# bgconley/cadence-rag

Hardware: AMD Instinct MI355X
Metric: queries/sec @ recall@10=1.0 (exact cosine top-10, 1024-d fp32 corpus) (higher is better)
Workload: dtype f32; 1 GPU; BASELINE configs[1]: brute-force cosine top-10, 100000x1024 fp32 corpus on one GPU, 64 queries/step resident in HBM; rows_per_gpu=100000, rows_total=100000, dim=1024, k=10, parallelism=1 GPU, rounds=1, arithmetic=fp16-MFMA prefilter (proven bound) + exact fp32 rescoring, api=crag_index_search_async (in stream order), hbm_bytes_per_corpus_row=6156

## Files before the change

### cadence_rag_amd/csrc/crag_api.hip

```cpp

#include <hip/hip_runtime.h>
#include <stdarg.h>
#include <stdint.h>
#include <stdio.h>
#include <stdlib.h>
#include <string.h>

#include <mutex>
#include <new>
#include <vector>

#include "../../include/crag_dense.h"
#include "crag_kernels.h"

namespace {

thread_local char g_err[512] = "";

int fail(int code, const char *fmt, ...) {
    va_list ap;
    va_start(ap, fmt);
    vsnprintf(g_err, sizeof(g_err), fmt, ap);
    va_end(ap);
    return code;
}

#define HIP_TRY(expr)                                                                          \
    do {                                                                                       \
        hipError_t e_ = (expr);                                                                \
        if (e_ != hipSuccess)                                                                  \
            return fail(CRAG_EHIP, "%s failed: %s (%s:%d)", #expr, hipGetErrorString(e_),      \
                        __FILE__, __LINE__);                                                   \
    } while (0)

bool is_device_ptr(const void *p) {
    if (!p) return false;
    hipPointerAttribute_t attr;
    memset(&attr, 0, sizeof(attr));
    hipError_t e = hipPointerGetAttributes(&attr, p);
    if (e != hipSuccess) {
        (void)hipGetLastError();
        return false;
    }
    return attr.type == hipMemoryTypeDevice || attr.type == hipMemoryTypeManaged;
}

struct DevBuf {
    void *p = nullptr;
    size_t bytes = 0;
    int ensure(size_t need) {
        if (need <= bytes) return CRAG_OK;
        if (p) (void)hipFree(p);
        p = nullptr;
        bytes = 0;
        size_t want = need + need / 4;
        hipError_t e = hipMalloc(&p, want);
        if (e != hipSuccess) {
            p = nullptr;
            return fail(CRAG_ENOMEM, "hipMalloc(%zu) failed: %s", want, hipGetErrorString(e));
        }
        bytes = want;
        return CRAG_OK;
    }
    void release() {
        if (p) (void)hipFree(p);
        p = nullptr;
        bytes = 0;
    }
};

struct EvSet {
    hipEvent_t e0, e1a, e1, e2, e3;
};

}

struct crag_index {
    int device = 0;
    int dim = 0;
    int64_t capacity = 0;
    int64_t cap_rows = 0;
    int64_t size = 0;
    int n_cu = 0;
    float *corpus = nullptr;
    _Float16 *corpus16 = nullptr;
    float *inv_norm = nullptr;
    int64_t *ids = nullptr;
    static constexpr int MAX_WS = 8;
    struct Workspace {
        hipStream_t stream = nullptr;
        bool in_use = false;
        DevBuf partial, gbound;
        DevBuf a32, a16, qinv, pf_gbound, pf_cand, pf_count, pf_flags, pf_xkeys, pf_xids, pf_xcount, pf_xticket;
        hipEvent_t done = nullptr;
        uint32_t seq = 0;
        bool done_recorded = false;
        bool dirty = false;
        uint64_t last_use = 0;
    } ws[MAX_WS];
    static constexpr int MAX_PIPE = 4;
    int n_pipe = 3;
    hipStream_t pipe[MAX_PIPE] = {nullptr, nullptr, nullptr, nullptr};
    hipEvent_t pipe_fork[MAX_PIPE] = {nullptr, nullptr, nullptr, nullptr}, pipe_done[MAX_PIPE] = {nullptr, nullptr, nullptr, nullptr};
    bool pipe_pending[MAX_PIPE] = {false, false, false, false};
    unsigned pipe_next = 0;
    uint64_t use_clock = 0;
    bool record_done = false;
    int64_t last_id = INT64_MIN;
    bool env_no_wide = false, env_no_reverse = false, env_unpipelined = false, env_no_prefilter = false, env_no_rsplit = false;
    int env_pf_derive_lag = 2, env_pf_read_lag = 4;
    int env_pf_nt = -1;
    int64_t nt_above_bytes = 1536ll << 20;
    bool irregular = false;
    uint32_t *irregular_dev = nullptr;
    unsigned long long *pf_stats = nullptr;
    unsigned long long *phase_trace = nullptr;
    const char *last_scan_kernel = "";
    DevBuf stage_q, stage_rows, stage_ids, stage_mask, stage_out, scratch;
    int64_t edit_chunk_rows = 16384;
    DevBuf edit_bounce, edit_srcpos, edit_mask, edit_prefix, edit_newpos;
    std::mutex mu;
    int pass_parity = 0;
    int64_t env_fail_after_scan = 0;
    int64_t pf_searches = 0;
    int profiling = 0;
    int64_t prof_calls = 0;
    std::vector<EvSet> ev_pool;
    size_t ev_used = 0;
};

static_assert(crag_index::MAX_WS == crag::PF_STAT_WS, "one block of statistics records per workspace");

namespace {

struct DeviceGuard {
    int prev = -1;
    bool ok = false;
    explicit DeviceGuard(int dev) {
        if (hipGetDevice(&prev) != hipSuccess) prev = -1;
        ok = (hipSetDevice(dev) == hipSuccess);
    }
    ~DeviceGuard() {
        if (prev >= 0) (void)hipSetDevice(prev);
    }
};

int scan_groups(const crag_index *ix) {
    int64_t n8 = (ix->size + 7) / 8;
    int64_t g = ix->n_cu;
    if (g > n8) g = n8;
    if (g < 1) g = 1;
    return (int)g;
}

int search_device(crag_index *ix, const float *d_queries, int nq, int k, const uint8_t *d_mask,
                  int64_t mask_stride, int64_t *d_out_ids, float *d_out_scores, int32_t *d_out_counts,
                  hipStream_t st) {
    if (nq <= 0) return CRAG_OK;
    int q_blocks = (nq + 31) / 32;
    const bool wide = (nq > 32) && !ix->env_no_wide;
    if (wide) q_blocks = ((nq + 63) / 64) * 2;
    const int nq_pad = q_blocks * 32;
    const int G = scan_groups(ix);
    const bool prefilter = !ix->env_no_prefilter && !ix->irregular &&
                           ix->size >= (int64_t)G * crag::PF_MIN_ROWS_PER_GROUP && (wide || nq <= 32);
    int rc;
    crag_index::Workspace *ws = nullptr;
    for (auto &w : ix->ws)
        if (w.in_use && w.stream == st) ws = &w;
    if (!ws)
        for (auto &w : ix->ws)
            if (!w.in_use) {
                w.in_use = true;
                w.stream = st;
                ws = &w;
                if (&w == &ix->ws[crag_index::MAX_WS - 1]) ix->record_done = true;
                break;
            }
    if (!ws) {
        for (auto &w : ix->ws)
            if (!ws || w.last_use < ws->last_use) ws = &w;
        if (ws->done_recorded && !ws->dirty) {
            HIP_TRY(hipStreamWaitEvent(st, ws->done, 0));
        } else {
            HIP_TRY(hipDeviceSynchronize());
        }
        ix->record_done = true;
        ws->stream = st;
    }
    ws->last_use = ++ix->use_clock;
    if ((rc = ws->partial.ensure((size_t)q_blocks * G * 32 * (size_t)k * sizeof(uint2)))) return rc;
    {
        const size_t gb_bytes = (size_t)q_blocks * 32 * crag::GB_CELLS * sizeof(uint32_t);
        if (gb_bytes > ws->gbound.bytes) {
            if ((rc = ws->gbound.ensure(gb_bytes))) return rc;
            HIP_TRY(hipMemsetAsync(ws->gbound.p, 0, ws->gbound.bytes, st));
        }
    }
    if ((rc = ws->a32.ensure((size_t)nq_pad * crag::DIM * sizeof(float)))) return rc;
    if ((rc = ws->qinv.ensure((size_t)nq_pad * sizeof(float)))) return rc;
    const int cap = (k > 104 && nq_pad <= 128) ? 32768 : 8192;
    const int rsplit = (k <= 32 || ix->env_no_rsplit) ? 1 : (nq <= 16 ? 8 : (nq <= 128 ? 4 : 1));
    if (prefilter) {
        if ((rc = ws->a16.ensure((size_t)nq_pad * crag::DIM * 2))) return rc;
        {
            const size_t need = (size_t)(ix->n_cu + nq_pad) * crag::PF_BOUND_CELLS * sizeof(uint32_t);
            if (need > ws->pf_gbound.bytes) {
                if ((rc = ws->pf_gbound.ensure(need))) return rc;
                HIP_TRY(hipMemsetAsync(ws->pf_gbound.p, 0, ws->pf_gbound.bytes, st));
            }
        }
        if ((rc = ws->pf_cand.ensure((size_t)nq_pad * cap * sizeof(uint2)))) return rc;
        if (rsplit > 1) {
            const size_t slots = (size_t)nq_pad * 8;
            if ((rc = ws->pf_xkeys.ensure(slots * CRAG_MAX_K * sizeof(uint64_t)))) return rc;
            if ((rc = ws->pf_xids.ensure(slots * CRAG_MAX_K * sizeof(int64_t)))) return rc;
            if ((rc = ws->pf_xcount.ensure(slots * sizeof(uint2)))) return rc;
            const size_t tneed = (size_t)nq_pad * sizeof(uint32_t);
            if (tneed > ws->pf_xticket.bytes) {
                if ((rc = ws->pf_xticket.ensure(tneed))) return rc;
                HIP_TRY(hipMemsetAsync(ws->pf_xticket.p, 0, ws->pf_xticket.bytes, st));
            }
        }
        {
            const size_t need = (size_t)nq_pad * sizeof(uint32_t);
            if (need > ws->pf_count.bytes) {
                if ((rc = ws->pf_count.ensure(need))) return rc;
                HIP_TRY(hipMemsetAsync(ws->pf_count.p, 0, ws->pf_count.bytes, st));
            }
            if (ws->pf_flags.bytes == 0) {
                if ((rc = ws->pf_flags.ensure(4 * sizeof(uint32_t)))) return rc;
                HIP_TRY(hipMemsetAsync(ws->pf_flags.p, 0, ws->pf_flags.bytes, st));
            }
        }
        if (ws->dirty) {
            HIP_TRY(hipMemsetAsync(ws->pf_gbound.p, 0, ws->pf_gbound.bytes, st));
            HIP_TRY(hipMemsetAsync(ws->pf_count.p, 0, ws->pf_count.bytes, st));
            HIP_TRY(hipMemsetAsync(ws->pf_flags.p, 0, ws->pf_flags.bytes, st));
            if (ws->pf_xticket.p) HIP_TRY(hipMemsetAsync(ws->pf_xticket.p, 0, ws->pf_xticket.bytes, st));
            ws->dirty = false;
        }
    }

    const int64_t rows_per_g = (ix->size + G - 1) / G + 64;
    if (rows_per_g * (int64_t)(crag::DIM * 4) >= (int64_t)0x7ff00000)
        return fail(CRAG_EINVAL, "index too large for one device scan window (%lld rows)",
                    (long long)ix->size);

    EvSet *ev = nullptr;
    if (ix->profiling > 0 && (ix->prof_calls++ % ix->profiling) == ix->profiling / 2) {
        if (ix->ev_used == ix->ev_pool.size()) {
            EvSet t;
            HIP_TRY(hipEventCreate(&t.e0));
            HIP_TRY(hipEventCreate(&t.e1a));
            HIP_TRY(hipEventCreate(&t.e1));
            HIP_TRY(hipEventCreate(&t.e2));
            HIP_TRY(hipEventCreate(&t.e3));
            ix->ev_pool.push_back(t);
        }
        ev = &ix->ev_pool[ix->ev_used++];
        HIP_TRY(hipEventRecord(ev->e0, st));
    }

    crag::PrepParams pp;
    pp.queries = d_queries;
    pp.nq = nq;
    pp.dim = ix->dim;
    pp.qinv = (float *)ws->qinv.p;
    pp.a32 = (float *)ws->a32.p;
    pp.a16 = prefilter ? (_Float16 *)ws->a16.p : nullptr;
    HIP_TRY(crag::launch_prep_queries(pp, nq_pad, st));

    crag::ScanParams sp;
    sp.wide = wide ? 1 : 0;
    sp.corpus = ix->corpus;
    sp.inv_norm = ix->inv_norm;
    sp.queries = d_queries;
    sp.a32 = (const float *)ws->a32.p;
    sp.qinv = (const float *)ws->qinv.p;
    sp.gate = nullptr;
    sp.dim = ix->dim;
    sp.mask = (const uint32_t *)d_mask;
    sp.mask_stride_w = mask_stride / 4;
    sp.partial = (uint2 *)ws->partial.p;
    sp.gbound = (uint32_t *)ws->gbound.p;
    sp.n_rows = ix->size;
    sp.cap_rows = ix->cap_rows;
    sp.nq = nq;
    sp.k = k;
    sp.G = G;
    sp.nb = k < crag::GB_CELLS ? k : crag::GB_CELLS;
    sp.pub_rank = (k + sp.nb - 1) / sp.nb - 1;
    sp.reverse = ix->pass_parity;
    ix->pass_parity ^= 1;
    if (ix->env_no_reverse) sp.reverse = 0;
    sp.unpipelined = (ix->env_unpipelined && !prefilter) ? 1 : 0;
    sp.piece_shift = crag::crag_piece_shift(ix->corpus16 != nullptr);

    crag::MergeParams mp;
    mp.partial = (const uint2 *)ws->partial.p;
    mp.ids = ix->ids;
    mp.gbound = (uint32_t *)ws->gbound.p;
    mp.id_base = 0;
    mp.out_ids = d_out_ids;
    mp.out_scores = d_out_scores;
    mp.out_counts = d_out_counts;
    mp.k = k;
    mp.G = G;

    if (ev) {
        HIP_TRY(hipEventRecord(ev->e1a, st));
        HIP_TRY(hipEventRecord(ev->e1, st));
    }
    if (prefilter) {
        crag::PfParams fp;
        fp.corpus = ix->corpus;
        fp.corpus16 = ix->corpus16;
        fp.inv_norm = ix->inv_norm;
        fp.a16 = (const _Float16 *)ws->a16.p;
        fp.qinv = (const float *)ws->qinv.p;
        fp.mask = (const uint32_t *)d_mask;
        fp.mask_stride_w = mask_stride / 4;
        fp.gbound_idle = (const uint32_t *)ws->pf_gbound.p;
        fp.gbound = (uint32_t *)ws->pf_gbound.p + (size_t)ix->n_cu * crag::PF_BOUND_CELLS;
        fp.cand = (uint2 *)ws->pf_cand.p;
        fp.count = (uint32_t *)ws->pf_count.p;
        fp.flags = (uint32_t *)ws->pf_flags.p;
        if (++ws->seq == 0u) ws->seq = 1u;
        fp.seq = ws->seq;
        fp.n_rows = ix->size;
        fp.nq = nq;
        fp.k = k;
        fp.G = G;
        fp.reverse = sp.reverse;
        fp.sets = k <= 24 ? 1 : (k <= 56 ? 2 : 4);
        fp.pub0 = (k + fp.sets - 1) / fp.sets >= 27 ? 8 : fp.sets;
        fp.cap = cap;
        fp.derive_lag = ix->corpus16 ? ix->env_pf_derive_lag : 1;
        fp.read_lag = ix->corpus16 ? ix->env_pf_read_lag : 2;
        {
            const int64_t streamed = ix->size * (int64_t)crag::DIM * 2;
            fp.nt = !ix->corpus16 ? 0 : (ix->env_pf_nt >= 0 ? ix->env_pf_nt : (streamed > ix->nt_above_bytes ? 1 : 0));
        }
        const int nqb = wide ? 2 : 1;
        ws->dirty = true;
        HIP_TRY(crag::launch_prefilter(fp, nqb, nq_pad / (32 * nqb), st, &ix->last_scan_kernel));
        if (ix->env_fail_after_scan > 0 && ++ix->pf_searches == ix->env_fail_after_scan)
            return fail(CRAG_EHIP, "injected failure behind the scan launch (CRAG_TEST_FAIL_AFTER_SCAN)");
        if (ev) HIP_TRY(hipEventRecord(ev->e2, st));
        crag::FinParams fin;
        fin.corpus = ix->corpus;
        fin.inv_norm = ix->inv_norm;
        fin.a32 = (const float *)ws->a32.p;
        fin.qinv = (const float *)ws->qinv.p;
        fin.cand = (const uint2 *)ws->pf_cand.p;
        fin.count = (uint32_t *)ws->pf_count.p;
        fin.gbound = fp.gbound;
        fin.flags = (const uint32_t *)ws->pf_flags.p;
        fin.seq = fp.seq;
        fin.ids = ix->ids;
        fin.out_ids = d_out_ids;
        fin.out_scores = d_out_scores;
        fin.out_counts = d_out_counts;
        fin.stats = ix->pf_stats + (size_t)(ws - ix->ws) * (crag::PF_STAT_SLOTS / crag_index::MAX_WS) * 3;
        fin.k = k;
        fin.cap = cap;
        fin.merge = mp;
        fin.nq = nq;
        fin.rsplit = rsplit;
        fin.xkeys = nullptr;
        fin.xids = nullptr;
        fin.xcount = nullptr;
        fin.xticket = nullptr;
        if (fin.rsplit > 1) {
            fin.xkeys = (uint64_t *)ws->pf_xkeys.p;
            fin.xids = (int64_t *)ws->pf_xids.p;
            fin.xcount = (uint2 *)ws->pf_xcount.p;
            fin.xticket = (uint32_t *)ws->pf_xticket.p;
        }
        sp.wide = 0;
        sp.gate = nullptr;
        sp.unpipelined = 1;
        fin.scan = sp;
        fin.fb_blocks = G * ((nq + 31) / 32);
        fin.fb_done = (uint32_t *)ws->pf_flags.p + 1;
        fin.trace = ix->phase_trace;
        HIP_TRY(crag::launch_finalize(fin, st));
        ws->dirty = false;
    } else {
        HIP_TRY(crag::launch_scan(sp, q_blocks, st, &ix->last_scan_kernel));
        if (ev) HIP_TRY(hipEventRecord(ev->e2, st));
        HIP_TRY(crag::launch_merge_partials(mp, nq, st));
    }
    if (ev) HIP_TRY(hipEventRecord(ev->e3, st));
    ws->done_recorded = ix->record_done;
    if (ix->record_done) HIP_TRY(hipEventRecord(ws->done, st));
    return CRAG_OK;
}

int check_search_args(const crag_index *ix, const void *queries, int nq, int k, const void *mask,
                      int64_t mask_stride, const void *out_ids, const void *out_scores,
// ... 9 lines not shown
            return fail(CRAG_EINVAL, "mask_stride must be 0 or a multiple of 4 >= %lld (got %lld)",
                        (long long)need, (long long)mask_stride);
        if (((uintptr_t)mask) & 3) return fail(CRAG_EINVAL, "row_mask must be 4-byte aligned");
    }
    return CRAG_OK;
}

}

extern "C" {

const char *crag_last_error(void) { return g_err; }

void crag_set_error_(const char *msg) { snprintf(g_err, sizeof(g_err), "%s", msg ? msg : ""); }

const char *crag_version(void) { return "cadence-rag_amd dense lane 0.1 (gfx950)"; }

int crag_device_count(void) {
    int n = 0;
    if (hipGetDeviceCount(&n) != hipSuccess) {
        (void)hipGetLastError();
        return 0;
    }
    return n;
}

int crag_index_create(int device, int dim, int64_t capacity, crag_index **out) {
    if (!out) return fail(CRAG_EINVAL, "out is NULL");
    *out = nullptr;
    if (dim <= 0 || dim > CRAG_DIM) return fail(CRAG_EINVAL, "dim must be in [1, %d] (got %d)", CRAG_DIM, dim);
    if (capacity <= 0) return fail(CRAG_EINVAL, "capacity must be > 0 (got %lld)", (long long)capacity);
    int ndev = crag_device_count();
    if (ndev <= 0) return fail(CRAG_ENODEV, "no HIP device visible");
    if (device < 0 || device >= ndev) return fail(CRAG_EINVAL, "device %d out of range [0, %d)", device, ndev);
    DeviceGuard guard(device);
    if (!guard.ok) return fail(CRAG_EHIP, "hipSetDevice(%d) failed", device);
    hipDeviceProp_t prop;
    HIP_TRY(hipGetDeviceProperties(&prop, device));
    if (strncmp(prop.gcnArchName, "gfx950", 6) != 0)
        return fail(CRAG_ENODEV, "device %d is %s; this library is built for gfx950 only", device,
                    prop.gcnArchName);
    crag_index *ix = new (std::nothrow) crag_index();
    if (!ix) return fail(CRAG_ENOMEM, "out of host memory");
    ix->device = device;
    ix->dim = dim;
    ix->capacity = capacity;
    ix->cap_rows = ((capacity + 31) / 32) * 32;
    ix->n_cu = prop.multiProcessorCount;
    const size_t cbytes = (size_t)ix->cap_rows * crag::DIM * sizeof(float);
    hipError_t e;
    if ((e = hipMalloc((void **)&ix->corpus, cbytes)) != hipSuccess ||
        (e = hipMalloc((void **)&ix->inv_norm, (size_t)ix->cap_rows * sizeof(float))) != hipSuccess ||
        (e = hipMalloc((void **)&ix->ids, (size_t)ix->cap_rows * sizeof(int64_t))) != hipSuccess) {
        int rc = fail(CRAG_ENOMEM, "hipMalloc for %lld rows failed: %s", (long long)ix->cap_rows,
                      hipGetErrorString(e));
        crag_index_destroy(ix);
        return rc;
    }
    if ((e = hipMemset(ix->inv_norm, 0, (size_t)ix->cap_rows * sizeof(float))) != hipSuccess ||
        (e = hipMemset(ix->corpus, 0, cbytes)) != hipSuccess) {
        int rc = fail(CRAG_EHIP, "hipMemset failed: %s", hipGetErrorString(e));
        crag_index_destroy(ix);
        return rc;
    }
    for (auto &w : ix->ws)
        if ((e = hipEventCreateWithFlags(&w.done, hipEventDisableTiming)) != hipSuccess) {
            int rc = fail(CRAG_EHIP, "hipEventCreate failed: %s", hipGetErrorString(e));
            crag_index_destroy(ix);
            return rc;
        }
    ix->env_no_wide = getenv("CRAG_NO_WIDE") != nullptr;
    ix->env_no_reverse = getenv("CRAG_NO_REVERSE") != nullptr;
    ix->env_unpipelined = getenv("CRAG_UNPIPELINED") != nullptr;
    ix->env_no_prefilter = getenv("CRAG_NO_PREFILTER") != nullptr;
    ix->env_no_rsplit = getenv("CRAG_NO_RSPLIT") != nullptr;
    if (const char *v = getenv("CRAG_PF_NT")) ix->env_pf_nt = atoi(v) ? 1 : 0;
    if (const char *v = getenv("CRAG_PF_LAGS")) {
        int d = 0, r = 0;
        if (sscanf(v, "%d,%d", &d, &r) == 2 && d >= 1 && r > d && r <= 4) {
            ix->env_pf_derive_lag = d;
            ix->env_pf_read_lag = r;
        }
    }
    if (const char *v = getenv("CRAG_TEST_FAIL_AFTER_SCAN")) ix->env_fail_after_scan = atoll(v);
    if (const char *v = getenv("CRAG_PIPE_STREAMS")) {
        const int n = atoi(v);
        if (n >= 1 && n <= crag_index::MAX_PIPE) ix->n_pipe = n;
    }
    if (const char *v = getenv("CRAG_EDIT_CHUNK_ROWS")) {
        const long long c = atoll(v);
        if (c >= 32 && c % 32 == 0 && c <= ((long long)1 << 24)) ix->edit_chunk_rows = c;
    }
    if (const char *v = getenv("CRAG_PF_NT_ABOVE_MB")) ix->nt_above_bytes = (int64_t)atoll(v) << 20;
    if (!ix->env_no_prefilter && getenv("CRAG_NO_FP16_MIRROR") == nullptr) {
        const size_t mbytes = (size_t)ix->cap_rows * crag::DIM * sizeof(_Float16);
        if ((e = hipMalloc((void **)&ix->corpus16, mbytes)) != hipSuccess ||
            (e = hipMemset(ix->corpus16, 0, mbytes)) != hipSuccess) {
            int rc = fail(CRAG_ENOMEM, "hipMalloc for the fp16 mirror of %lld rows failed: %s", (long long)ix->cap_rows,
                          hipGetErrorString(e));
            crag_index_destroy(ix);
            return rc;
        }
    }
    if ((e = hipMalloc((void **)&ix->irregular_dev, sizeof(uint32_t))) != hipSuccess ||
        (e = hipMalloc((void **)&ix->pf_stats, crag::PF_STAT_SLOTS * 3 * sizeof(unsigned long long))) != hipSuccess ||
        (e = hipMemset(ix->irregular_dev, 0, sizeof(uint32_t))) != hipSuccess ||
        (e = hipMemset(ix->pf_stats, 0, crag::PF_STAT_SLOTS * 3 * sizeof(unsigned long long))) != hipSuccess) {
        int rc = fail(CRAG_ENOMEM, "hipMalloc for the index state failed: %s", hipGetErrorString(e));
        crag_index_destroy(ix);
        return rc;
    }
    if (getenv("CRAG_PHASE_TRACE") != nullptr) {
        if ((e = hipMalloc((void **)&ix->phase_trace, 128 * sizeof(unsigned long long))) != hipSuccess ||
            (e = hipMemset(ix->phase_trace, 0, 128 * sizeof(unsigned long long))) != hipSuccess) {
            int rc = fail(CRAG_ENOMEM, "hipMalloc for the phase trace failed: %s", hipGetErrorString(e));
            crag_index_destroy(ix);
            return rc;
        }
    }
    *out = ix;
    return CRAG_OK;
}

int crag_index_destroy(crag_index *ix) {
    if (!ix) return CRAG_OK;
    DeviceGuard guard(ix->device);
    (void)hipDeviceSynchronize();
    for (auto &t : ix->ev_pool) {
        (void)hipEventDestroy(t.e0);
        (void)hipEventDestroy(t.e1a);
        (void)hipEventDestroy(t.e1);
        (void)hipEventDestroy(t.e2);
        (void)hipEventDestroy(t.e3);
    }
    if (ix->irregular_dev) (void)hipFree(ix->irregular_dev);
    if (ix->phase_trace) (void)hipFree(ix->phase_trace);
    for (int i = 0; i < crag_index::MAX_PIPE; ++i) {
        if (ix->pipe_fork[i]) (void)hipEventDestroy(ix->pipe_fork[i]);
        if (ix->pipe_done[i]) (void)hipEventDestroy(ix->pipe_done[i]);
        if (ix->pipe[i]) (void)hipStreamDestroy(ix->pipe[i]);
    }
    if (ix->pf_stats) (void)hipFree(ix->pf_stats);
    if (ix->corpus) (void)hipFree(ix->corpus);
    if (ix->corpus16) (void)hipFree(ix->corpus16);
    if (ix->inv_norm) (void)hipFree(ix->inv_norm);
    if (ix->ids) (void)hipFree(ix->ids);
    for (auto &w : ix->ws) {
        w.partial.release();
        w.gbound.release();
        w.a32.release();
        w.a16.release();
        w.qinv.release();
        w.pf_gbound.release();
        w.pf_cand.release();
        w.pf_count.release();
        w.pf_flags.release();
        w.pf_xkeys.release();
        w.pf_xids.release();
        w.pf_xcount.release();
        w.pf_xticket.release();
        if (w.done) (void)hipEventDestroy(w.done);
    }
    ix->stage_q.release();
    ix->stage_rows.release();
    ix->stage_ids.release();
    ix->stage_mask.release();
    ix->stage_out.release();
    ix->scratch.release();
    ix->edit_bounce.release();
    ix->edit_srcpos.release();
    ix->edit_mask.release();
    ix->edit_prefix.release();
    ix->edit_newpos.release();
    delete ix;
    return CRAG_OK;
}

int64_t crag_index_size(const crag_index *ix) { return ix ? ix->size : -1; }
int64_t crag_index_capacity(const crag_index *ix) { return ix ? ix->capacity : -1; }
int crag_index_dim(const crag_index *ix) { return ix ? ix->dim : -1; }

static int recompute_irregular(crag_index *ix) {
    HIP_TRY(hipMemsetAsync(ix->irregular_dev, 0, sizeof(uint32_t), 0));
    HIP_TRY(crag::launch_irregular_flag(ix->inv_norm, ix->size, ix->irregular_dev, 0));
    uint32_t flag = 0;
    HIP_TRY(hipMemcpy(&flag, ix->irregular_dev, sizeof(flag), hipMemcpyDeviceToHost));
    ix->irregular = flag != 0;
    return CRAG_OK;
}

static int store_rows_locked(crag_index *ix, int64_t pos, const float *rows, int64_t n) {
    const int64_t CH = 65536;
    const bool dev = is_device_ptr(rows);
    for (int64_t o = 0; o < n; o += CH) {
        const int64_t m = (n - o < CH) ? (n - o) : CH;
        const float *src = rows + (size_t)o * ix->dim;
        if (!dev) {
            int rc = ix->stage_rows.ensure((size_t)m * ix->dim * sizeof(float));
            if (rc) return rc;
            HIP_TRY(hipMemcpy(ix->stage_rows.p, src, (size_t)m * ix->dim * sizeof(float), hipMemcpyHostToDevice));
            src = (const float *)ix->stage_rows.p;
        }
        HIP_TRY(crag::launch_store_rows(src, ix->dim, pos + o, m, ix->corpus, ix->inv_norm, ix->irregular_dev, ix->corpus16, 0));
        if (!dev) HIP_TRY(hipStreamSynchronize(0));
    }
    HIP_TRY(hipStreamSynchronize(0));
    if (!ix->irregular) {
        uint32_t flag = 0;
        HIP_TRY(hipMemcpy(&flag, ix->irregular_dev, sizeof(flag), hipMemcpyDeviceToHost));
        ix->irregular = flag != 0;
    }
    return CRAG_OK;
}

int crag_index_add(crag_index *ix, const float *rows, const int64_t *ids, int64_t n) {
    if (!ix) return fail(CRAG_EINVAL, "index is NULL");
    if (n < 0) return fail(CRAG_EINVAL, "n must be >= 0");
    if (n == 0) return CRAG_OK;
    if (!rows) return fail(CRAG_EINVAL, "rows is NULL");
    std::lock_guard<std::mutex> lk(ix->mu);
    if (ix->size + n > ix->capacity)
        return fail(CRAG_ENOMEM, "capacity exceeded: size %lld + %lld > %lld", (long long)ix->size,
                    (long long)n, (long long)ix->capacity);
    if (ix->size + n >= (int64_t)0xfffffff0ll) return fail(CRAG_ENOMEM, "more than 2^32 rows per index");
    DeviceGuard guard(ix->device);
    const int64_t pos = ix->size;
    int64_t new_last;
    if (!ids) {
        if (pos <= ix->last_id)
            return fail(CRAG_EINVAL, "implicit ids would start at %lld, not above the largest stored id %lld",
                        (long long)pos, (long long)ix->last_id);
        new_last = pos + n - 1;
    } else if (is_device_ptr(ids)) {
        int rc0 = ix->scratch.ensure(sizeof(unsigned long long));
        if (rc0) return rc0;
        HIP_TRY(hipMemsetAsync(ix->scratch.p, 0, sizeof(unsigned long long), 0));
        HIP_TRY(crag::launch_check_ids(ids, n, ix->last_id, (unsigned long long *)ix->scratch.p, 0));
        unsigned long long bad = 0;
        HIP_TRY(hipMemcpy(&bad, ix->scratch.p, sizeof(bad), hipMemcpyDeviceToHost));
// ... 642 lines not shown
```

### cadence_rag_amd/csrc/crag_kernels.h

```cpp
#pragma once
#include <hip/hip_runtime.h>
#include <stdint.h>

#include "crag_arch.h"

namespace crag {

constexpr int TILE_ROWS = 32;
constexpr int DIM = 1024;
constexpr int TILE_FLOATS = TILE_ROWS * DIM;
constexpr int SCAN_WAVES = 8;
constexpr int SCAN_THREADS = SCAN_WAVES * 64;
constexpr int KSLICE = DIM / SCAN_WAVES;
constexpr int GB_CELLS = 32;

struct ScanParams {
    const float *corpus;
    const float *inv_norm;
    const float *queries;
    const float *a32;
    const float *qinv;
    const uint32_t *gate;
    int wide;
    const uint32_t *mask;
    int64_t mask_stride_w;
    uint2 *partial;
    uint32_t *gbound;
    int64_t n_rows;
    int64_t cap_rows;
    int nq;
    int dim;
    int k;
    int G;
    int nb;
    int pub_rank;
    int reverse;
    int unpipelined;
    int piece_shift;
};

struct MergeParams {
    const uint2 *partial;
    const int64_t *ids;
    uint32_t *gbound;
    int64_t id_base;
    int64_t *out_ids;
    float *out_scores;
    int32_t *out_counts;
    int k;
    int G;
};

constexpr int PF_BOUND_CELLS = 160;
constexpr int PF_STAT_WS = 8;
constexpr int PF_STAT_SLOTS = 2048;
constexpr int PF_MIN_ROWS_PER_GROUP = 128;

struct PrepParams {
    const float *queries;
    int nq, dim;
    float *qinv;
    float *a32;
    _Float16 *a16;
};

struct PfParams {
    const float *corpus;
    const _Float16 *corpus16;
    const float *inv_norm;
    const _Float16 *a16;
    const float *qinv;
    const uint32_t *mask;
    int64_t mask_stride_w;
    uint32_t *gbound;
    const uint32_t *gbound_idle;
    uint2 *cand;
    uint32_t *count;
    uint32_t *flags;
    uint32_t seq;
    int64_t n_rows;
    int nq, k, G, reverse;
    int sets;
    int pub0;
    int nt;
    int derive_lag, read_lag;
    int cap;
};

struct FinParams {
    const float *corpus;
    const float *inv_norm;
    const float *a32;
    const float *qinv;
    const uint2 *cand;
    uint32_t *count;
    uint32_t *gbound;
    const uint32_t *flags;
    uint32_t seq;
    const int64_t *ids;
    int64_t *out_ids;
    float *out_scores;
    int32_t *out_counts;
    unsigned long long *stats;
    int k, cap;
    int nq;
    int rsplit;
    uint64_t *xkeys;
    int64_t *xids;
    uint2 *xcount;
    uint32_t *xticket;
    int fb_blocks;
    uint32_t *fb_done;
    unsigned long long *trace;

    ScanParams scan;
    MergeParams merge;
};

struct XMergeParams {
    const int64_t *ids;
    const float *scores;
    const int32_t *counts;
    int64_t *out_ids;
    float *out_scores;
    int32_t *out_counts;
    int64_t stride_ids, stride_scores, stride_counts;
    int n_lists;
    int nq;
    int k;
};

hipError_t launch_scan(const ScanParams &p, int q_blocks, hipStream_t st, const char **kernel_name);
hipError_t launch_prep_queries(const PrepParams &p, int nq_pad, hipStream_t st);
hipError_t launch_prefilter(const PfParams &p, int nqb, int passes, hipStream_t st, const char **kernel_name);
hipError_t launch_finalize(const FinParams &p, hipStream_t st);
hipError_t launch_merge_partials(const MergeParams &p, int nq, hipStream_t st);
hipError_t launch_merge_results(const XMergeParams &p, hipStream_t st);
hipError_t launch_store_rows(const float *rows, int dim, int64_t pos, int64_t n, float *corpus,
                             float *inv_norm, uint32_t *irregular, _Float16 *mirror, hipStream_t st);
hipError_t launch_load_rows(const float *corpus, int dim, int64_t pos, int64_t n, float *rows, int piece_shift,
                            hipStream_t st);
inline int crag_piece_shift(bool has_mirror) { return has_mirror ? 5 : 2; }
hipError_t launch_count_eligible(const float *inv_norm, int64_t n, const uint32_t *mask,
                                 unsigned long long *out, hipStream_t st);
hipError_t launch_check_ids(const int64_t *ids, int64_t n, int64_t prev, unsigned long long *out_bad,
                            hipStream_t st);
hipError_t launch_fill_ids(int64_t *ids, int64_t pos, int64_t n, int64_t first, hipStream_t st);

struct RowStore {
    float *corpus;
    _Float16 *mirror;
    float *inv_norm;
    int64_t *ids;
};
hipError_t launch_lookup_ids(const int64_t *stored, int64_t size, const int64_t *ids, int64_t n, int64_t *pos,
                             int add_index, uint32_t *drop, unsigned long long *found, hipStream_t st);
hipError_t launch_remove_srcpos(const uint32_t *keep, const uint32_t *prefix, int64_t n_words, int64_t d0, int64_t m,
                                int64_t *srcpos, hipStream_t st);
hipError_t launch_insert_srcpos(const int64_t *newpos, int64_t n_new, int64_t d0, int64_t m, int64_t *srcpos,
                                hipStream_t st);
hipError_t launch_move_rows(const RowStore &index, const RowStore &bounce, const int64_t *srcpos, int64_t d0, int64_t m,
                            hipStream_t st);
hipError_t launch_store_rows_at(const float *rows, int dim, const int64_t *dstpos, const int64_t *new_ids, int64_t n,
                                const RowStore &index, uint32_t *irregular, hipStream_t st);
hipError_t launch_clear_rows(const RowStore &index, int64_t pos, int64_t n, hipStream_t st);
hipError_t launch_irregular_flag(const float *inv_norm, int64_t n, uint32_t *flag, hipStream_t st);

constexpr int BM25_RANGE = 16384;
constexpr int BM25_MAX_Q = 64;
// ... 26 lines not shown
```

### cadence_rag_amd/csrc/crag_search.hip

```cpp

#include <hip/hip_runtime.h>
#include <stdint.h>

#include <type_traits>

#include "crag_kernels.h"
#include "crag_layout.h"

namespace crag {

typedef float f32x16 __attribute__((ext_vector_type(16)));

__device__ __forceinline__ uint32_t f2ord(float f) {
    uint32_t u = __float_as_uint(f);
    return (u & 0x80000000u) ? ~u : (u | 0x80000000u);
}
__device__ __forceinline__ float ord2f(uint32_t u) {
    u = (u & 0x80000000u) ? (u & 0x7fffffffu) : ~u;
    return __uint_as_float(u);
}
__device__ __forceinline__ uint64_t mk64(uint32_t hi, uint32_t lo) {
    return ((uint64_t)hi << 32) | lo;
}

// ... 1253 lines not shown
        const int64_t id = p.ids[(size_t)l * p.stride_ids + src];
        if (pos < cnt) {
            const int idx = atomicAdd(&s_cnt, 1);
            s_sc[idx] = f2ord(sc);
            s_id[idx] = id;
        }
    }
    __syncthreads();
    const int C = s_cnt;
    const int count = C < k ? C : k;
    for (int e = tid; e < C; e += MERGE_THREADS) {
        const uint32_t ms = s_sc[e];
        const int64_t mi = s_id[e];
        int rank = 0;
        for (int i = 0; i < C; ++i) {
            const uint32_t os = s_sc[i];
            rank += (os > ms || (os == ms && s_id[i] < mi)) ? 1 : 0;
        }
        if (rank < k) {
            p.out_scores[(size_t)q * k + rank] = ord2f(ms);
            p.out_ids[(size_t)q * k + rank] = mi;
        }
    }
    for (int r = count + tid; r < k; r += MERGE_THREADS) {
        p.out_scores[(size_t)q * k + r] = __uint_as_float(0x7fc00000u);
        p.out_ids[(size_t)q * k + r] = -1;
    }
    if (tid == 0) p.out_counts[q] = count;
}

template <int PS>
__global__ __launch_bounds__(256) void store_rows_kernel(const float *rows, int dim, int64_t pos,
                                                         float *corpus, float *inv_norm, uint32_t *irregular,
                                                         _Float16 *mirror) {
    const int64_t i = blockIdx.x;
    store_row<PS>(rows + (size_t)i * dim, dim, pos + i, corpus, inv_norm, irregular, mirror);
}

template <int PS>
__global__ __launch_bounds__(256) void load_rows_kernel(const float *corpus, int dim, int64_t pos,
                                                        float *rows) {
    const int64_t i = blockIdx.x;
    const int kq = threadIdx.x;
    const int64_t row = pos + i;
    const float *src = corpus + (size_t)(row >> 5) * TILE_FLOATS + ((size_t)(kq >> PS) * 32 + (row & 31)) * (4 << PS) + (kq & ((1 << PS) - 1)) * 4;
    const f32x4 v = *reinterpret_cast<const f32x4 *>(src);
    float *dst = rows + (size_t)i * dim;
#pragma unroll
    for (int c = 0; c < 4; ++c)
        if (4 * kq + c < dim) dst[4 * kq + c] = v[c];
}

__global__ __launch_bounds__(256) void count_eligible_kernel(const float *inv_norm, int64_t n,
                                                             const uint32_t *mask,
                                                             unsigned long long *out) {
    unsigned long long c = 0;
    for (int64_t i = (int64_t)blockIdx.x * blockDim.x + threadIdx.x; i < n;
         i += (int64_t)gridDim.x * blockDim.x) {
        bool ok = inv_norm[i] > 0.f;
        if (ok && mask) ok = (mask[i >> 5] >> (i & 31)) & 1u;
        c += ok ? 1 : 0;
    }
    for (int o = 32; o > 0; o >>= 1) c += __shfl_xor(c, o);
    if ((threadIdx.x & 63) == 0 && c) atomicAdd(out, c);
}

__global__ void fill_ids_kernel(int64_t *ids, int64_t pos, int64_t n, int64_t first) {
    const int64_t i = (int64_t)blockIdx.x * blockDim.x + threadIdx.x;
    if (i < n) ids[pos + i] = first + i;
}

constexpr float PF_DELTA = 1.25e-3f;
constexpr int PF_FLUSH_ABOVE = 768;
constexpr int PF_STAGE = PF_FLUSH_ABOVE + 2048;
constexpr int PF_PER = (PF_STAGE + SCAN_THREADS - 1) / SCAN_THREADS;
constexpr int PF_TAU_CELL = 128;
constexpr int PF_STASH_MIRROR = 4;
constexpr int PF_STASH_ROWS = 2;

typedef _Float16 f16x8 __attribute__((ext_vector_type(8)));
typedef _Float16 f16x2 __attribute__((ext_vector_type(2)));
typedef float f32x2 __attribute__((ext_vector_type(2)));

__global__ __launch_bounds__(256) void prep_queries_kernel(PrepParams p) {
    __shared__ double sh[4];
    const int q = blockIdx.x, t = threadIdx.x;
    const f32x4 v = load_query_quad(p.queries, p.dim, q, p.nq, t);
    const float qinv = canonical_qinv(v, q < p.nq, sh);
    if (t == 0) p.qinv[q] = qinv;
    const int qb = q >> 5, i = q & 31, w = t >> 5, d = (4 * t) & 127;
    {
        const int sidx = d >> 3, h = (d >> 2) & 1;
        reinterpret_cast<f32x4 *>(p.a32)[((size_t)(qb * SCAN_WAVES + w) * 16 + sidx) * 64 + h * 32 + i] = v;
    }
    if (p.a16) {
        const int t8 = d >> 4, g = (d >> 3) & 1, h = (d >> 2) & 1;
        f32x2 lo = {v[0] * qinv, v[1] * qinv}, hi = {v[2] * qinv, v[3] * qinv};
        const f16x2 l2 = __builtin_convertvector(lo, f16x2), h2 = __builtin_convertvector(hi, f16x2);
        _Float16 *dst = p.a16 + ((((size_t)(qb * SCAN_WAVES + w) * 8 + t8) * 64 + h * 32 + i) * 8 + 4 * g);
        typedef _Float16 f16x4 __attribute__((ext_vector_type(4)));
        *reinterpret_cast<f16x4 *>(dst) = f16x4{l2[0], l2[1], h2[0], h2[1]};
    }
}

template <int X>
__device__ __forceinline__ uint32_t dpp_xor(uint32_t v, int lane) {
    if constexpr (X == 1) return (uint32_t)__builtin_amdgcn_mov_dpp((int)v, 0xB1, 0xF, 0xF, true);
    else if constexpr (X == 2) return (uint32_t)__builtin_amdgcn_mov_dpp((int)v, 0x4E, 0xF, 0xF, true);
    else if constexpr (X == 3) return (uint32_t)__builtin_amdgcn_mov_dpp((int)v, 0x1B, 0xF, 0xF, true);
    else if constexpr (X == 7) return (uint32_t)__builtin_amdgcn_mov_dpp((int)v, 0x141, 0xF, 0xF, true);
    else if constexpr (X == 15) return (uint32_t)__builtin_amdgcn_mov_dpp((int)v, 0x140, 0xF, 0xF, true);
    else if constexpr (X == 8) return (uint32_t)__builtin_amdgcn_mov_dpp((int)v, 0x128, 0xF, 0xF, true);
    else if constexpr (X == 4) {
        const uint32_t up = (uint32_t)__builtin_amdgcn_mov_dpp((int)v, 0x12C, 0xF, 0xF, true);
        const uint32_t dn = (uint32_t)__builtin_amdgcn_mov_dpp((int)v, 0x124, 0xF, 0xF, true);
        return (lane & 4) ? dn : up;
    } else return swz_xor<X>(v);
}

__device__ __forceinline__ uint32_t sort32_desc_u32(uint32_t v, int lane) {
#define CRAG_CX(X_, BIT_)                                              \
    {                                                                  \
        const uint32_t o_ = dpp_xor<X_>(v, lane);                      \
        const bool mx_ = !(lane & BIT_);                               \
        v = mx_ ? (o_ > v ? o_ : v) : (o_ < v ? o_ : v);               \
    }
    CRAG_CX(1, 1) CRAG_CX(3, 2) CRAG_CX(1, 1) CRAG_CX(7, 4) CRAG_CX(2, 2) CRAG_CX(1, 1) CRAG_CX(15, 8) CRAG_CX(4, 4)
    CRAG_CX(2, 2) CRAG_CX(1, 1) CRAG_CX(31, 16) CRAG_CX(8, 8) CRAG_CX(4, 4) CRAG_CX(2, 2) CRAG_CX(1, 1)
#undef CRAG_CX
    return v;
}

template <class F>
__device__ __forceinline__ uint32_t wave_reduce_u32(uint32_t v, int lane, F f) {
    v = f(v, dpp_xor<1>(v, lane));
    v = f(v, dpp_xor<2>(v, lane));
    v = f(v, dpp_xor<4>(v, lane));
    v = f(v, dpp_xor<8>(v, lane));
    const auto r16 = __builtin_amdgcn_permlane16_swap(v, v, false, false);
    v = f(r16[0], r16[1]);
    const auto r32 = __builtin_amdgcn_permlane32_swap(v, v, false, false);
    return f(r32[0], r32[1]);
}

template <int NQB>
struct PfLds {
    typedef float slab_t __attribute__((ext_vector_type(2 * NQB)));
    slab_t slab[2][SCAN_WAVES][SCAN_WAVES][64];
    uint2 stage[PF_STAGE];
    float qthr[32 * NQB];
    uint32_t qcount[32 * NQB], qbase[32 * NQB], qfill[32 * NQB];
    uint32_t n_stage;
    uint32_t need[NQB];
    uint32_t want_flush[2][SCAN_WAVES];
};

template <int NQB>
struct PfOwner {
    int ql0;
    int qg0;
    uint32_t okmask;
};

template <int NQB>
__device__ __forceinline__ void pf_stage(PfLds<NQB> &L, const PfOwner<NQB> &o, const float (&sc)[2 * NQB],
                                         const bool (&pass)[2 * NQB], uint32_t row_in_window, uint32_t *flags, uint32_t seq) {
#pragma unroll
    for (int e = 0; e < 2 * NQB; ++e) {
        if (pass[e]) {
            const uint32_t slot = atomicAdd(&L.n_stage, 1u);
            if (slot < (uint32_t)PF_STAGE) {
                L.stage[slot] = make_uint2(f2ord(sc[e]), (row_in_window << 6) | (uint32_t)(o.ql0 + e));
            } else {
                *flags = seq;
            }
        }
    }
}

template <int NQB, bool LAST>
__device__ __forceinline__ void pf_sift(const PfParams &p, PfLds<NQB> &L, int64_t window_row0) {
    __syncthreads();
    const uint32_t n = L.n_stage < (uint32_t)PF_STAGE ? L.n_stage : (uint32_t)PF_STAGE;
    const int tid = threadIdx.x;
    if (LAST && n == 0u) return;
    uint2 ent[PF_PER];
    bool keep[PF_PER];
#pragma unroll
    for (int i = 0; i < PF_PER; ++i) {
        const uint32_t idx = (uint32_t)tid + (uint32_t)i * SCAN_THREADS;
        keep[i] = false;
        if (idx < n) {
            ent[i] = L.stage[idx];
            keep[i] = ord2f(ent[i].x) >= L.qthr[ent[i].y & 63u];
        }
    }
    if (tid < 32 * NQB) {
        L.qcount[tid] = 0u;
        L.qfill[tid] = 0u;
    }
    __syncthreads();
    if (tid == 0) L.n_stage = 0u;
    __syncthreads();
#pragma unroll
    for (int i = 0; i < PF_PER; ++i)
        if (keep[i]) {
            atomicAdd(&L.qcount[ent[i].y & 63u], 1u);
            if (!LAST) L.stage[atomicAdd(&L.n_stage, 1u)] = ent[i];
        }
    __syncthreads();
    if constexpr (!LAST) {
        const uint32_t kept = L.n_stage;
        __syncthreads();
        if (kept <= (uint32_t)(PF_FLUSH_ABOVE / 2)) return;
    }
    if (tid < 32 * NQB) {
        const uint32_t cnt = L.qcount[tid];
        const int qg = (int)blockIdx.y * (32 * NQB) + tid;
        L.qbase[tid] = cnt ? atomicAdd(&p.count[qg], cnt) : 0u;
    }
    __syncthreads();
#pragma unroll
    for (int i = 0; i < PF_PER; ++i)
        if (keep[i]) {
            const uint32_t ql = ent[i].y & 63u;
            const uint32_t pos = L.qbase[ql] + atomicAdd(&L.qfill[ql], 1u);
            const int qg = (int)blockIdx.y * (32 * NQB) + (int)ql;
            if (pos < (uint32_t)p.cap) {
                p.cand[(size_t)qg * p.cap + pos] = make_uint2(ent[i].x, (uint32_t)(window_row0 + (int64_t)(ent[i].y >> 6)));
            } else {
                p.flags[0] = p.seq;
            }
        }
    if (LAST) return;
    __syncthreads();
    if (tid == 0) L.n_stage = 0u;
    __syncthreads();
}


__device__ __forceinline__ int pf_next_pub(int after, int n_tiles, int read_lag) {
    const int last = n_tiles >= 12 ? n_tiles - 4 : -1;
    const int np = after < 0 ? 0 : (after == 0 ? read_lag + 1 : after * 4 + 3);
    if (after < last && np + (np >> 2) >= last) return last;
    return (np < n_tiles) ? np : (1 << 30);
}

template <int NQB, int SETS, bool MIRROR, bool NT>
__global__ __launch_bounds__(SCAN_THREADS) void prefilter_kernel(PfParams p) {
    constexpr int RPO = 2 * NQB;
    constexpr int AUX = NT ? 2 : 0;
    __shared__ PfLds<NQB> L;
    ScanCtx c;
    c.lane = threadIdx.x & 63;
    c.w = __builtin_amdgcn_readfirstlane((int)(threadIdx.x >> 6));
    c.g = blockIdx.x;
    c.qb = blockIdx.y;
    c.j = c.lane & 31;
    c.h = c.lane >> 5;
    c.reverse = p.reverse != 0;
    constexpr int PS = PS_SMALL;
    c.lane_off = (uint32_t)(c.w * (KSLICE * 32 * 4) + c.j * (16 << PS) + c.h * 16);
    {
        const uint32_t nt = (uint32_t)((p.n_rows + 31) >> 5), G = (uint32_t)p.G, g = (uint32_t)c.g;
        const uint32_t qt = nt / G, rt = nt - qt * G;
        const uint32_t t0 = qt * g + (rt * g) / G, t1 = qt * (g + 1) + (rt * (g + 1)) / G;
        c.t_begin = t0;
        c.n_tiles = (int)(t1 - t0);
        c.r_begin = (int64_t)t0 * 32;
        c.r_end = (int64_t)t1 * 32 < p.n_rows ? (int64_t)t1 * 32 : p.n_rows;
    }
    const int lane = c.lane, w = c.w, j = c.j, h = c.h;

    constexpr int NB = MIRROR ? 8 : 16;
    constexpr uint32_t TILE_BYTES = MIRROR ? TILE_FLOATS * 2 : TILE_FLOATS * 4;
    const char *wg_base = MIRROR ? reinterpret_cast<const char *>(p.corpus16) + (size_t)c.t_begin * TILE_BYTES
                                 : reinterpret_cast<const char *>(p.corpus) + (size_t)c.t_begin * TILE_BYTES;
    const __amdgpu_buffer_rsrc_t rsrc = __builtin_amdgcn_make_buffer_rsrc(
        const_cast<char *>(wg_base), 0, (int)((uint32_t)c.n_tiles * TILE_BYTES), 0x00020000);
    const uint32_t lane_off = MIRROR ? (uint32_t)(w * (8 * 1024) + lane * 16) : c.lane_off;
    auto voff = [&](int step) -> uint32_t {
        const int t = tile_of(c, step);
        const int64_t r = (c.t_begin + t) * 32 + j;
        const bool valid = (step < c.n_tiles) && (r >= c.r_begin) && (r < c.r_end);
        return valid ? (uint32_t)t * TILE_BYTES + lane_off : 0x80000000u;
    };
    u32x4 b[NB];
    {
        const uint32_t v0 = voff(0);
#pragma unroll
        for (int s = 0; s < NB; ++s) b[s] = __builtin_amdgcn_raw_buffer_load_b128(rsrc, v0 + (MIRROR ? (uint32_t)s * 1024u : b_soff<PS>(s)), 0, AUX);
    }
    f16x8 a[NQB][8];
    PfOwner<NQB> o;
    {
        const int R = w * RPO, qb = R >> 4, r = R & 15;
        o.ql0 = qb * 32 + (r & 3) + 8 * (r >> 2) + 4 * h;
        o.qg0 = (int)blockIdx.y * (32 * NQB) + o.ql0;
        o.okmask = 0u;
    }
    {
#pragma unroll
        for (int qb = 0; qb < NQB; ++qb) {
            const f16x8 *af = reinterpret_cast<const f16x8 *>(p.a16) +
                              ((size_t)(((int)blockIdx.y * NQB + qb) * SCAN_WAVES + w) * 8) * 64 + lane;
#pragma unroll
            for (int t8 = 0; t8 < 8; ++t8) a[qb][t8] = af[t8 * 64];
        }
        typedef float qv_t __attribute__((ext_vector_type(RPO)));
        const qv_t qi = *reinterpret_cast<const qv_t *>(p.qinv + o.qg0);
#pragma unroll
        for (int e = 0; e < RPO; ++e)
            if (o.qg0 + e < p.nq && qi[e] > 0.f) o.okmask |= 1u << e;
    }
    if (threadIdx.x < 32 * NQB) L.qthr[threadIdx.x] = -__builtin_inff();
    if (threadIdx.x < NQB) L.need[threadIdx.x] = 0u;
    if (threadIdx.x == 0) L.n_stage = 0u;
    constexpr int PF_STASH = MIRROR ? PF_STASH_MIRROR : PF_STASH_ROWS;
    float stash[PF_STASH][RPO];
#pragma unroll
    for (int t = 0; t < PF_STASH; ++t)
#pragma unroll
        for (int e = 0; e < RPO; ++e) stash[t][e] = __uint_as_float(0x7fc00000u);
    float thr[RPO];
    uint32_t tau[RPO];
    uint32_t lmax[RPO][SETS];
    uint32_t dirty = 0u;
#pragma unroll
    for (int e = 0; e < RPO; ++e) {
        thr[e] = -__builtin_inff();
        tau[e] = 0u;
#pragma unroll
        for (int s = 0; s < SETS; ++s) lmax[e][s] = 0u;
    }
    float inv_cur = 1.f;
    if (!MIRROR && c.n_tiles > 0) inv_cur = p.inv_norm[(c.t_begin + tile_of(c, 0)) * 32 + j];
    __builtin_amdgcn_s_waitcnt(0x0F70);
    __syncthreads();

    const int k_base = p.k / SETS, k_rem = p.k % SETS;
    const f32x16 zero16 = f32x16{0, 0, 0, 0, 0, 0, 0, 0, 0, 0, 0, 0, 0, 0, 0, 0};
    uint32_t *const gb_row = p.gbound + (size_t)o.qg0 * PF_BOUND_CELLS + j;
    const uint32_t *const idle_row = p.gbound_idle + (size_t)c.g * PF_BOUND_CELLS + j;

    auto load_taus = [&](uint32_t (&tq)[RPO]) {
#pragma unroll
        for (int e = 0; e < RPO; ++e) {
            const bool live = (o.okmask >> e) & 1u;
            tq[e] = __hip_atomic_load(live ? gb_row - j + e * PF_BOUND_CELLS + PF_TAU_CELL : idle_row - j + PF_TAU_CELL,
                                      __ATOMIC_RELAXED, __HIP_MEMORY_SCOPE_AGENT);
        }
    };
    auto take_taus = [&](const uint32_t (&tq)[RPO]) {
#pragma unroll
        for (int e = 0; e < RPO; ++e)
            if (tq[e] > tau[e]) {
                tau[e] = tq[e];
                thr[e] = ord2f(tq[e]) - 2.f * PF_DELTA;
                if (j == 0) L.qthr[o.ql0 + e] = thr[e];
            }
    };
    auto any_without_bound = [&]() -> bool {
        bool none = false;
#pragma unroll
        for (int e = 0; e < RPO; ++e) none = none || (((o.okmask >> e) & 1u) && tau[e] == 0u);
        return __builtin_amdgcn_ballot_w64(none) != 0ull;
    };
    constexpr int DS = SETS >= 2 ? SETS / 2 : 1;
    auto load_cells = [&](int dq, uint32_t (&cell)[DS]) {
        const uint32_t *rec = p.gbound + (size_t)((int)blockIdx.y * (32 * NQB) + dq) * PF_BOUND_CELLS;
#pragma unroll
        for (int i = 0; i < DS; ++i)
            cell[i] = __hip_atomic_load(rec + (SETS >= 2 ? 2 * i + h : 0) * 32 + j, __ATOMIC_RELAXED, __HIP_MEMORY_SCOPE_AGENT);
    };
    auto derive_cells = [&](int dq, const uint32_t (&cell)[DS]) {
        uint32_t t = 0xffffffffu;
#pragma unroll
        for (int i = 0; i < DS; ++i) {
            const uint32_t sorted = sort32_desc_u32(cell[i], lane);
            const int sset = SETS >= 2 ? 2 * i + h : 0;
            const int ks = k_base + (sset < k_rem ? 1 : 0);
            const uint32_t kth = (uint32_t)__shfl((int)sorted, (lane & 32) | (ks - 1));
            t = kth < t ? kth : t;
        }
        if constexpr (SETS >= 2) {
            const uint32_t other = (uint32_t)__shfl((int)t, lane ^ 32);
            t = other < t ? other : t;
        }
        if (lane == 0 && t != 0u)
            (void)__hip_atomic_fetch_max(p.gbound + (size_t)((int)blockIdx.y * (32 * NQB) + dq) * PF_BOUND_CELLS + PF_TAU_CELL, t,
                                         __ATOMIC_RELAXED, __HIP_MEMORY_SCOPE_AGENT);
    };
    auto derive_own = [&]() {
#pragma unroll
        for (int e = 0; e < RPO; ++e) {
            const bool live = (o.okmask >> e) & 1u;
            uint32_t t = 0xffffffffu;
#pragma unroll
            for (int s = 0; s < SETS; ++s) {
                const uint32_t v = __hip_atomic_load(live ? gb_row + e * PF_BOUND_CELLS + s * 32 : idle_row + s * 32,
// ... 762 lines not shown
```

Baseline: 1.349 million queries/sec.

## Fuse query preparation into prefilter kernel with cross-block ready flags

Query normalisation and fp16 packing now run inside the prefilter kernel instead of a separate prep launch. Each block prepares a strided share of its query group's queries, publishes them through per-query sequence-stamped ready flags, and then spins with a bounded timeout. Any query still missing after the timeout is prepared redundantly by the waiting block. This removes one kernel launch and its serialization gap per search, at the cost of spin-waiting, extra fences, a new ready buffer and memset handling.

```diff
diff --git a/cadence_rag_amd/csrc/crag_api.hip b/cadence_rag_amd/csrc/crag_api.hip
--- a/cadence_rag_amd/csrc/crag_api.hip
+++ b/cadence_rag_amd/csrc/crag_api.hip
@@ -91,7 +91,7 @@
         hipStream_t stream = nullptr;
         bool in_use = false;
         DevBuf partial, gbound;
-        DevBuf a32, a16, qinv, pf_gbound, pf_cand, pf_count, pf_flags, pf_xkeys, pf_xids, pf_xcount, pf_xticket;
+        DevBuf a32, a16, qinv, pf_gbound, pf_cand, pf_count, pf_flags, pf_ready, pf_xkeys, pf_xids, pf_xcount, pf_xticket;
         hipEvent_t done = nullptr;
         uint32_t seq = 0;
         bool done_recorded = false;
@@ -121,6 +121,7 @@
     DevBuf edit_bounce, edit_srcpos, edit_mask, edit_prefix, edit_newpos;
     std::mutex mu;
     int pass_parity = 0;
+    int env_pf_prep = 1;
     int64_t env_fail_after_scan = 0;
     int64_t pf_searches = 0;
     int profiling = 0;
@@ -232,11 +233,16 @@
                 if ((rc = ws->pf_flags.ensure(4 * sizeof(uint32_t)))) return rc;
                 HIP_TRY(hipMemsetAsync(ws->pf_flags.p, 0, ws->pf_flags.bytes, st));
             }
+            if (need > ws->pf_ready.bytes) {
+                if ((rc = ws->pf_ready.ensure(need))) return rc;
+                HIP_TRY(hipMemsetAsync(ws->pf_ready.p, 0, ws->pf_ready.bytes, st));
+            }
         }
         if (ws->dirty) {
             HIP_TRY(hipMemsetAsync(ws->pf_gbound.p, 0, ws->pf_gbound.bytes, st));
             HIP_TRY(hipMemsetAsync(ws->pf_count.p, 0, ws->pf_count.bytes, st));
             HIP_TRY(hipMemsetAsync(ws->pf_flags.p, 0, ws->pf_flags.bytes, st));
+            HIP_TRY(hipMemsetAsync(ws->pf_ready.p, 0, ws->pf_ready.bytes, st));
             if (ws->pf_xticket.p) HIP_TRY(hipMemsetAsync(ws->pf_xticket.p, 0, ws->pf_xticket.bytes, st));
             ws->dirty = false;
         }
@@ -269,7 +275,8 @@
     pp.qinv = (float *)ws->qinv.p;
     pp.a32 = (float *)ws->a32.p;
     pp.a16 = prefilter ? (_Float16 *)ws->a16.p : nullptr;
-    HIP_TRY(crag::launch_prep_queries(pp, nq_pad, st));
+    const int pf_prep = prefilter ? ix->env_pf_prep : 0;
+    if (!pf_prep) HIP_TRY(crag::launch_prep_queries(pp, nq_pad, st));
 
     crag::ScanParams sp;
     sp.wide = wide ? 1 : 0;
@@ -317,6 +324,9 @@
         fp.corpus = ix->corpus;
         fp.corpus16 = ix->corpus16;
         fp.inv_norm = ix->inv_norm;
+        fp.prep_in = pp;
+        fp.prep = pf_prep;
+        fp.ready = (uint32_t *)ws->pf_ready.p;
         fp.a16 = (const _Float16 *)ws->a16.p;
         fp.qinv = (const float *)ws->qinv.p;
         fp.mask = (const uint32_t *)d_mask;
@@ -492,6 +502,8 @@
             ix->env_pf_read_lag = r;
         }
     }
+    if (getenv("CRAG_SEPARATE_PREP") != nullptr) ix->env_pf_prep = 0;
+    else if (getenv("CRAG_TEST_SELF_PREP") != nullptr) ix->env_pf_prep = 2;
     if (const char *v = getenv("CRAG_TEST_FAIL_AFTER_SCAN")) ix->env_fail_after_scan = atoll(v);
     if (const char *v = getenv("CRAG_PIPE_STREAMS")) {
         const int n = atoi(v);
@@ -565,6 +577,7 @@
         w.pf_cand.release();
         w.pf_count.release();
         w.pf_flags.release();
+        w.pf_ready.release();
         w.pf_xkeys.release();
         w.pf_xids.release();
         w.pf_xcount.release();
diff --git a/cadence_rag_amd/csrc/crag_kernels.h b/cadence_rag_amd/csrc/crag_kernels.h
--- a/cadence_rag_amd/csrc/crag_kernels.h
+++ b/cadence_rag_amd/csrc/crag_kernels.h
@@ -85,6 +85,9 @@
     int nt;
     int derive_lag, read_lag;
     int cap;
+    int prep;
+    PrepParams prep_in;
+    uint32_t *ready;
 };
 
 struct FinParams {
diff --git a/cadence_rag_amd/csrc/crag_search.hip b/cadence_rag_amd/csrc/crag_search.hip
--- a/cadence_rag_amd/csrc/crag_search.hip
+++ b/cadence_rag_amd/csrc/crag_search.hip
@@ -1359,11 +1359,10 @@
 typedef _Float16 f16x2 __attribute__((ext_vector_type(2)));
 typedef float f32x2 __attribute__((ext_vector_type(2)));
 
-__global__ __launch_bounds__(256) void prep_queries_kernel(PrepParams p) {
-    __shared__ double sh[4];
-    const int q = blockIdx.x, t = threadIdx.x;
+__device__ __forceinline__ void prep_query(const PrepParams &p, int q, int t, double *sh) {
     const f32x4 v = load_query_quad(p.queries, p.dim, q, p.nq, t);
     const float qinv = canonical_qinv(v, q < p.nq, sh);
+    if (t >= 256) return;
     if (t == 0) p.qinv[q] = qinv;
     const int qb = q >> 5, i = q & 31, w = t >> 5, d = (4 * t) & 127;
     {
@@ -1378,6 +1377,11 @@
         typedef _Float16 f16x4 __attribute__((ext_vector_type(4)));
         *reinterpret_cast<f16x4 *>(dst) = f16x4{l2[0], l2[1], h2[0], h2[1]};
     }
+}
+
+__global__ __launch_bounds__(256) void prep_queries_kernel(PrepParams p) {
+    __shared__ double sh[4];
+    prep_query(p, (int)blockIdx.x, (int)threadIdx.x, sh);
 }
 
 template <int X>
@@ -1430,7 +1434,11 @@
     uint32_t n_stage;
     uint32_t need[NQB];
     uint32_t want_flush[2][SCAN_WAVES];
+    double prep_sh[4];
+    uint32_t prep_miss[2];
 };
+
+constexpr unsigned long long PF_READY_WAIT = 40000ull;
 
 template <int NQB>
 struct PfOwner {
@@ -1521,6 +1529,45 @@
     const int np = after < 0 ? 0 : (after == 0 ? read_lag + 1 : after * 4 + 3);
     if (after < last && np + (np >> 2) >= last) return last;
     return (np < n_tiles) ? np : (1 << 30);
+}
+
+template <int NQB>
+__device__ __forceinline__ void pf_prepare_queries(PrepParams pp, uint32_t *ready, uint32_t seq, int mode, int G,
+                                                double *sh, uint32_t *miss_s) {
+    constexpr int QP = 32 * NQB;
+    const int q0 = (int)blockIdx.y * QP, lane = threadIdx.x & 63;
+    const int w = __builtin_amdgcn_readfirstlane((int)(threadIdx.x >> 6));
+    auto prepare = [&](int q) {
+        prep_query(pp, q, (int)threadIdx.x, sh);
+        if (w < 4) __builtin_amdgcn_fence(__ATOMIC_RELEASE, "agent");
+        __syncthreads();
+        if (threadIdx.x == 0) __hip_atomic_store(ready + q, seq, __ATOMIC_RELAXED, __HIP_MEMORY_SCOPE_AGENT);
+    };
+    if (mode == 1)
+        for (int ql = (int)blockIdx.x; ql < QP; ql += G) prepare(q0 + ql);
+    if (w == 0) {
+        const unsigned long long wait = mode == 1 ? PF_READY_WAIT : 0ull;
+        const unsigned long long t0 = __builtin_amdgcn_s_memtime();
+        unsigned long long miss;
+        for (;;) {
+            const uint32_t r = lane < QP ? __hip_atomic_load(ready + q0 + lane, __ATOMIC_RELAXED, __HIP_MEMORY_SCOPE_AGENT) : seq;
+            miss = __builtin_amdgcn_ballot_w64(r != seq);
+            if (miss == 0ull || __builtin_amdgcn_s_memtime() - t0 >= wait) break;
+            __builtin_amdgcn_s_sleep(2);
+        }
+        if (lane == 0) {
+            miss_s[0] = (uint32_t)miss;
+            miss_s[1] = (uint32_t)(miss >> 32);
+        }
+        __builtin_amdgcn_fence(__ATOMIC_ACQUIRE, "agent");
+    }
+    __syncthreads();
+    const uint32_t m0 = __builtin_amdgcn_readfirstlane(miss_s[0]), m1 = __builtin_amdgcn_readfirstlane(miss_s[1]);
+    if (m0 | m1) {
+        for (int half = 0; half < 2; ++half)
+            for (uint32_t m = half ? m1 : m0; m; m &= m - 1u) prepare(q0 + half * 32 + __builtin_ctz(m));
+        __builtin_amdgcn_fence(__ATOMIC_ACQUIRE, "agent");
+    }
 }
 
 template <int NQB, int SETS, bool MIRROR, bool NT>
@@ -1576,6 +1623,10 @@
         o.qg0 = (int)blockIdx.y * (32 * NQB) + o.ql0;
         o.okmask = 0u;
     }
+    if (threadIdx.x < 32 * NQB) L.qthr[threadIdx.x] = -__builtin_inff();
+    if (threadIdx.x < NQB) L.need[threadIdx.x] = 0u;
+    if (threadIdx.x == 0) L.n_stage = 0u;
+    if (p.prep) pf_prepare_queries<NQB>(p.prep_in, p.ready, p.seq, p.prep, p.G, L.prep_sh, L.prep_miss);
     {
 #pragma unroll
         for (int qb = 0; qb < NQB; ++qb) {
@@ -1590,9 +1641,6 @@
         for (int e = 0; e < RPO; ++e)
             if (o.qg0 + e < p.nq && qi[e] > 0.f) o.okmask |= 1u << e;
     }
-    if (threadIdx.x < 32 * NQB) L.qthr[threadIdx.x] = -__builtin_inff();
-    if (threadIdx.x < NQB) L.need[threadIdx.x] = 0u;
-    if (threadIdx.x == 0) L.n_stage = 0u;
     constexpr int PF_STASH = MIRROR ? PF_STASH_MIRROR : PF_STASH_ROWS;
     float stash[PF_STASH][RPO];
 #pragma unroll
```

Result: slower. 1.121 million queries/sec (-16.9%).
